# mwhittaker/frankenpaxos

Measured on NVIDIA H100. Metric: committed slots/sec (simulated) at 1M in-flight slots, higher is better.
Workload: dtype int32

## Files before the change

### frankenpaxos_b200/_lib.py

```python
import ctypes as C
import os

from . import build as _build

_lib = None

SYMBOLS = [
    "fpx_abi_version", "fpx_strerror", "fpx_last_error", "fpx_create", "fpx_destroy", "fpx_reset",
    "fpx_proxyleader_arm", "fpx_acceptor_phase2a", "fpx_proxyleader_phase2b", "fpx_replica_chosen",
    "fpx_chosen_watermark", "fpx_quorum_eval", "fpx_snapshot_acceptor", "fpx_snapshot_log",
    "fpx_proxyleader_arm_dev", "fpx_acceptor_phase2a_dev", "fpx_proxyleader_phase2b_dev",
    "fpx_replica_chosen_dev", "fpx_replica_chosen_last_dev", "fpx_chosen_watermark_dev", "fpx_sync",
    "fpx_stream", "fpx_launch_count", "fpx_set_coop_ctas_per_sm", "fpx_step_dev", "fpx_step_kernel_ms", "fpx_step_arm_ms",
    "fpx_acceptor_phase1a", "fpx_leader_safe_values",
    "fpx_vm_client_request", "fpx_vm_phase2a", "fpx_vm_learn_chosen", "fpx_vm_skip", "fpx_vm_client_request_dev", "fpx_vm_phase2a_dev", "fpx_vm_step_dev",
    "fpx_mencius_arm_range", "fpx_mencius_acceptor_noop_range", "fpx_mencius_range_phase2b",
    "fpx_mencius_replica_chosen_range", "fpx_mencius_replica_range_first", "fpx_mencius_replica_range_fill",
    "fpx_wire_decode_inbound", "fpx_wire_decode_inbound_dev", "fpx_wire_encode_phase2b", "fpx_wire_encode_phase2b_dev",
    "fpx_wire_encode_nack", "fpx_wire_encode_chosen",
    "fpx_step_submit", "fpx_step_wait", "fpx_retire_below", "fpx_exchange_export", "fpx_exchange_attach", "fpx_exchange_attach_local", "fpx_exchange_epoch",
    "fpx_global_watermark", "fpx_global_watermark_dev",
    "fpx_conflict_index_create", "fpx_conflict_index_destroy", "fpx_conflict_index_put_snapshot", "fpx_conflict_index_batch",
    "fpx_depgraph_create", "fpx_depgraph_destroy", "fpx_depgraph_commit", "fpx_depgraph_update_executed", "fpx_depgraph_execute",
    "fpx_epaxos_stream", "fpx_epaxos_sync", "fpx_epaxos_lead_dev", "fpx_epaxos_preaccept_dev", "fpx_epaxos_accept_dev",
# ... 75 lines not shown
    L.fpx_wire_encode_nack.argtypes = [vp, vp, i32, vp, i32, vp, p(i64)]; L.fpx_wire_encode_nack.restype = i32
    L.fpx_wire_encode_chosen.argtypes = [vp, vp, i32, vp, vp, i32, vp, i32, vp, p(i64)]
    L.fpx_wire_encode_chosen.restype = i32
    L.fpx_step_dev.argtypes = [vp, vp, i32, vp, i32, vp, vp, vp, i32, vp, vp, i32]; L.fpx_step_dev.restype = i32
    L.fpx_vm_step_dev.argtypes = [vp, vp, i32, vp, i32, vp, vp, i32, vp, vp]; L.fpx_vm_step_dev.restype = i32
    L.fpx_step_kernel_ms.argtypes = [vp, i32, p(C.c_float), p(C.c_float)]; L.fpx_step_kernel_ms.restype = i32
    L.fpx_step_arm_ms.argtypes = [vp, i32, p(C.c_float)]; L.fpx_step_arm_ms.restype = i32
    L.fpx_sync.argtypes = [vp, p(SyncResult)]; L.fpx_sync.restype = i32
    L.fpx_set_coop_ctas_per_sm.argtypes = [vp, i32]; L.fpx_set_coop_ctas_per_sm.restype = i32
    L.fpx_stream.argtypes = [vp]; L.fpx_stream.restype = vp
    L.fpx_launch_count.argtypes = [vp]; L.fpx_launch_count.restype = i64
    L.fpx_retire_below.argtypes = [vp, i32]; L.fpx_retire_below.restype = i32
    L.fpx_step_submit.argtypes = [vp, vp, i32, vp, i32, vp, i32, vp, vp, vp]; L.fpx_step_submit.restype = i32
    L.fpx_step_wait.argtypes = [vp, p(i32), p(i32), p(i32), p(i32), p(i64)]; L.fpx_step_wait.restype = i32
    L.fpx_exchange_export.argtypes = [vp, vp]; L.fpx_exchange_export.restype = i32
    L.fpx_exchange_attach.argtypes = [vp, i32, vp]; L.fpx_exchange_attach.restype = i32
    L.fpx_exchange_attach_local.argtypes = [vp, i32, vp]; L.fpx_exchange_attach_local.restype = i32
    L.fpx_exchange_epoch.argtypes = [vp]; L.fpx_exchange_epoch.restype = C.c_uint32
    L.fpx_global_watermark_dev.argtypes = [vp, C.c_uint32, i32, vp, vp]; L.fpx_global_watermark_dev.restype = i32
    L.fpx_global_watermark.argtypes = [vp, C.c_uint32, i32, p(i32), vp]; L.fpx_global_watermark.restype = i32
    if hasattr(L, "fpx_debug_set_tally_path"):
        L.fpx_debug_set_tally_path.argtypes = [vp, i32]; L.fpx_debug_set_tally_path.restype = i32
        L.fpx_debug_last_tally_path.argtypes = [vp]; L.fpx_debug_last_tally_path.restype = i32
    if L.fpx_abi_version() != 1:
        raise ImportError("libfpx.so ABI version mismatch")
    _lib = L
    return L
```

### frankenpaxos_b200/csrc/fpx_acceptor.cuh

```cuda
#pragma once
#include "fpx_common.cuh"

namespace fpx {

struct VoteConflict { int32_t dst, slot; };

struct AcceptorParams {
  Geometry g;
  const int4* in;
  int32_t n;
  int4* out_p2b;
  int2* out_nack;
  unsigned long long* votes;
  int32_t* acc_round;
  int32_t* acc_max_voted;
  uint32_t* accept_bits;
  int32_t* g_agg;
  uint32_t* g_wacc;
  uint32_t parity;
  int32_t append;
  DevStatus* st;
  VoteConflict* conflicts;
};

constexpr int kAccUnroll = 4;
#ifndef FPX_AT
#define FPX_AT 1024
#endif
constexpr int kAT = FPX_AT;
constexpr int kAW = kAT / 32;
__device__ __forceinline__ int grp_of(int dst) { return dst >> 16; }

__device__ __forceinline__ int decode_p2a(const Geometry& g, const int4& rec, int& key, int& loc, int& vix) {
  key = -1; loc = -1; vix = -1;
  int grp = rec.w >> 16, acc = rec.w & 0xffff;
  if ((uint32_t)grp >= (uint32_t)g.groups || acc >= g.per_group) return FPX_ERR_BAD_ACCEPTOR;
  if ((uint32_t)rec.y > (uint32_t)FPX_MAX_ROUND) return FPX_ERR_ROUND_RANGE;
  int l = local_slot(g, rec.x);
  if (l < 0 && l != kLocalRetired) return FPX_ERR_SLOT_RANGE;
  int v = voter_index(g, grp, acc, rec.x);
  if (v < 0 || (g.protocol == FPX_MENCIUS && grp != expected_group(g, rec.x))) return FPX_ERR_BAD_ACCEPTOR;
  key = grp * g.per_group + acc; loc = l; vix = v;
  return 0;
}
__device__ __forceinline__ int decode_key(const Geometry& g, const int4& rec) {
  int grp = rec.w >> 16, acc = rec.w & 0xffff;
  if ((uint32_t)grp >= (uint32_t)g.groups || acc >= g.per_group) return -1;
  if ((uint32_t)rec.y > (uint32_t)FPX_MAX_ROUND) return -1;
  return grp * g.per_group + acc;
}
__device__ __noinline__ void acceptor_error(DevStatus* st, int code, int index) { report_error(st, code, index); }

template <bool kExact>
__device__ __forceinline__ void acceptor_apply(const AcceptorParams& P, int4* out_p2b, int2* out_nack, int wlo, int whi,
                                               int lane, int run, uint32_t pos_base, int* s_mv, uint32_t& wacc,
                                               uint32_t& wnack) {
  const Geometry& g = P.g;
  const unsigned full = 0xffffffffu;
  const unsigned long long pol_out = l2_policy_evict_first();
  for (int base = wlo; base < whi; base += 32 * kAccUnroll) {
    int4 rec[kAccUnroll];
    unsigned long long cell[kAccUnroll], old[kAccUnroll];
#pragma unroll
    for (int u = 0; u < kAccUnroll; ++u) {
      int i = base + u * 32 + lane;
      rec[u] = (i < whi) ? ld_cg(P.in + i) : make_int4(0, -1, 0, -1);
      cell[u] = 0; old[u] = 0;
    }
#pragma unroll
    for (int u = 0; u < kAccUnroll; ++u) {
      const int i0 = base + u * 32;
      if (i0 >= whi) break;
      const int i = i0 + lane;
      int key, loc, vix;
      bool valid = false;
      if (i < whi) {
        int err = decode_p2a(g, rec[u], key, loc, vix);
        if (err && !kExact) acceptor_error(P.st, err, i);
        valid = err == 0;
      }
      const int r = rec[u].y;
      int mn = __reduce_min_sync(full, valid ? r : INT_MAX);
      int mx = __reduce_max_sync(full, valid ? r : INT_MIN);
      if (mx == INT_MIN) {
        if (!kExact && lane == 0) P.accept_bits[i0 >> 5] = 0;
        continue;
      }
      int my_run = __shfl_sync(full, run, key & 31);
      int cur;
// ... 36 lines not shown
        uint32_t before = pos_base + wacc + __popc(b & lanemask_lt());
        if (accept) {
          st_stream(out_p2b + before, make_int4(rec[u].w >> 16, rec[u].w & 0xffff, rec[u].x, r));
        } else if (valid) {
          int ldr = r % g.num_leaders;
          if (g.protocol == FPX_MENCIUS) ldr += (grp_of(rec[u].w) / g.agroups) * g.num_leaders;
          st_stream2(out_nack + ((uint32_t)i - before), make_int2(ldr, cur));
        }
      }
      wacc += __popc(b);
    }
    if (!kExact) {
#pragma unroll
      for (int u = 0; u < kAccUnroll; ++u) {
        if ((old[u] >> 32) == (cell[u] >> 32) && old[u] != cell[u]) {
          uint32_t cidx = atomicAdd(&P.st->n_conflicts, 1u);
          if (cidx < (uint32_t)kMaxConflicts) P.conflicts[cidx] = VoteConflict{rec[u].w, rec[u].x};
        }
      }
    }
  }
}

__global__ void __launch_bounds__(kAT, 1024 / kAT) acceptor_phase2a_kernel(AcceptorParams P) {
  const Geometry& g = P.g;
  extern __shared__ int s_mv[];
  __shared__ int s_wagg[kAW][kMaxKeys];
  __shared__ int s_tmp[kAW][kMaxKeys];
  __shared__ int s_win;

  const unsigned full = 0xffffffffu;
  const int tid = threadIdx.x, lane = tid & 31, warp = tid >> 5;
  const int total_warps = gridDim.x * kAW;
  const int per = (((P.n + total_warps - 1) / total_warps) + 31) & ~31;
  const int gw = blockIdx.x * kAW + warp;
  const int wlo = (int)min((long long)P.n, (long long)gw * per);
  const int whi = (int)min((long long)P.n, (long long)wlo + per);
  uint32_t* nack_ctr = P.parity ? &P.st->nack_total : &P.st->pad[0];
  uint32_t* nack_other = P.parity ? &P.st->pad[0] : &P.st->nack_total;
  if (blockIdx.x == 0 && tid == 0) *nack_other = 0;
  const uint32_t base_p2b = P.append ? (uint32_t)__ldcg(&P.st->n_p2b) : 0u;
  const uint32_t base_nack = P.append ? (uint32_t)__ldcg(&P.st->n_nack) : 0u;
  int4* const out_p2b = P.out_p2b + base_p2b;
  int2* const out_nack = P.out_nack + base_nack;
  for (int k = 0; k < g.num_keys; ++k) s_mv[k * kAT + tid] = INT_MIN;
  FPX_MARK(P.st->t_acceptor, 0);

  const unsigned long long pol_keep = l2_policy_evict_last();
  int wagg = INT_MIN;
  for (int base = wlo; base < whi; base += 32 * kAccUnroll) {
    int4 rec[kAccUnroll];
#pragma unroll
    for (int u = 0; u < kAccUnroll; ++u) {
      int i = base + u * 32 + lane;
      rec[u] = (i < whi) ? ld_keep(P.in + i, pol_keep) : make_int4(0, -1, 0, -1);
    }
#pragma unroll
    for (int u = 0; u < kAccUnroll; ++u) {
      if (base + u * 32 >= whi) break;
      const int key = decode_key(g, rec[u]);
      const bool valid = key >= 0;
      const int r = rec[u].y;
      int mn = __reduce_min_sync(full, valid ? r : INT_MAX);
      int mx = __reduce_max_sync(full, valid ? r : INT_MIN);
      if (mx == INT_MIN) continue;
      if (mn == mx) {
        unsigned present = __reduce_or_sync(full, valid ? (1u << key) : 0u);
        if ((present >> lane) & 1u) wagg = max(wagg, mx);
      } else {
        unsigned remaining = __ballot_sync(full, valid);
        while (remaining) {
          int leader = __ffs(remaining) - 1;
          int kk = __shfl_sync(full, key, leader);
          bool mine = valid && key == kk;
          int m = __reduce_max_sync(full, mine ? r : INT_MIN);
          if (lane == kk) wagg = max(wagg, m);
          remaining &= ~__ballot_sync(full, mine);
        }
      }
    }
  }
  s_wagg[warp][lane] = wagg;
  __syncthreads();
  int cta_agg = INT_MIN;
  if (warp == 0) {
#pragma unroll
    for (int w = 0; w < kAW; ++w) cta_agg = max(cta_agg, s_wagg[w][lane]);
    __stcg(&P.g_agg[blockIdx.x * kMaxKeys + lane], cta_agg);
  }
  FPX_MARK(P.st->t_acceptor, 1);
  grid_sync(P.st);
  FPX_MARK(P.st->t_acceptor, 2);

  for (int k = 0; k < g.num_keys; ++k) {
    int v = INT_MIN;
    for (int c = tid; c < (int)blockIdx.x; c += kAT) v = max(v, __ldcg(&P.g_agg[c * kMaxKeys + k]));
    v = __reduce_max_sync(full, v);
    if (lane == 0) s_tmp[warp][k] = v;
  }
  __syncthreads();
  int cta_carry = INT_MIN;
  if (lane < g.num_keys) {
    cta_carry = __ldcg(&P.acc_round[lane]);
#pragma unroll
    for (int w = 0; w < kAW; ++w) cta_carry = max(cta_carry, s_tmp[w][lane]);
  }
  int run = cta_carry;
  for (int w = 0; w < warp; ++w) run = max(run, s_wagg[w][lane]);

  FPX_MARK(P.st->t_acceptor, 3);
  uint32_t wacc = 0, wnack = 0;
  acceptor_apply<false>(P, out_p2b, out_nack, wlo, whi, lane, run, 0u, s_mv, wacc, wnack);
  if (lane == 0) {
    __stcg(&P.g_wacc[gw], wacc);
    if (wnack) atomicAdd(nack_ctr, wnack);
  }
  __syncthreads();
  for (int k = warp; k < g.num_keys; k += kAW) {
    int m = INT_MIN;
#pragma unroll
    for (int t = lane; t < kAT; t += 32) m = max(m, s_mv[k * kAT + t]);
    m = __reduce_max_sync(full, m);
    if (lane == 0 && m != INT_MIN) atomicMax(&P.acc_max_voted[k], m);
  }
  FPX_MARK(P.st->t_acceptor, 4);
  grid_sync(P.st);
  FPX_MARK(P.st->t_acceptor, 5);

  if (blockIdx.x == gridDim.x - 1 && warp == 0 && lane < g.num_keys) {
    int tot = cta_carry;
#pragma unroll
    for (int w = 0; w < kAW; ++w) tot = max(tot, s_wagg[w][lane]);
    P.acc_round[lane] = tot;
  }
  const uint32_t total_nacks = __ldcg(nack_ctr);
  if (total_nacks == 0) {
    if (blockIdx.x == 0 && tid == 0) { P.st->n_p2b = (int)base_p2b + P.n; P.st->n_nack = (int)base_nack; }
  } else {
    uint32_t before = 0;
    for (int j = lane; j < gw; j += 32) before += __ldcg(&P.g_wacc[j]);
    before = __reduce_add_sync(full, before);
    uint32_t wacc2 = 0, wnack2 = 0;
    acceptor_apply<true>(P, out_p2b, out_nack, wlo, whi, lane, run, before, s_mv, wacc2, wnack2);
    if (gw == (int)gridDim.x * kAW - 1 && lane == 0) {
      P.st->n_p2b = (int)(base_p2b + before + wacc2);
      P.st->n_nack = (int)base_nack + P.n - (int)(before + wacc2);
    }
  }

  if (blockIdx.x != 0) return;
  uint32_t nc = __ldcg(&P.st->n_conflicts);
  if (nc == 0) return;
  if (nc > (uint32_t)kMaxConflicts) {
    if (tid == 0) { report_error(P.st, FPX_ERR_CONFLICT, 0); P.st->n_conflicts = 0; }
    return;
  }
  for (uint32_t cix = 0; cix < nc; ++cix) {
    int dst = P.conflicts[cix].dst, slot = P.conflicts[cix].slot;
    if (tid == 0) s_win = -1;
    __syncthreads();
    for (int j = tid; j < P.n; j += kAT) {
      int4 rr = P.in[j];
      if (rr.w == dst && rr.x == slot && ((__ldcg(&P.accept_bits[j >> 5]) >> (j & 31)) & 1u)) atomicMax(&s_win, j);
    }
    __syncthreads();
    if (tid == 0 && s_win >= 0) {
      int4 rr = P.in[s_win];
      int l = local_slot(g, slot);
      int v = voter_index(g, dst >> 16, dst & 0xffff, slot);
// ... 9 lines not shown
```

### frankenpaxos_b200/csrc/fpx_arm.cuh

```cuda
#pragma once
#include "fpx_common.cuh"
#include "fpx_ranges.cuh"

namespace fpx {

struct ArmConflict { int32_t slot, round; };

struct ArmParams {
  Geometry g;
  PLState pl;
  const int4* in;
  int32_t n;
  DevStatus* st;
  ArmConflict* conflicts;
  uint32_t* win_bits;
  unsigned long long* votes;
  int32_t vanilla;
  RangeTable rng;
  int32_t check_rng;
};

__device__ __forceinline__ void note_arm_conflict(const ArmParams& P, int slot, int round) {
  uint32_t c = atomicAdd(&P.st->n_arm_conflicts, 1u);
  if (c < (uint32_t)kMaxConflicts) P.conflicts[c] = ArmConflict{slot, round};
// ... 83 lines not shown
        int i = (c0 + u) * 32 + lane;
        rec[u] = (c0 + u < n_chunks && i < P.n) ? ld_stream(P.in + i) : make_int4(-1, 0, 0, 0);
      }
#pragma unroll
      for (int u = 0; u < kArmUnroll; ++u) {
        int i = (c0 + u) * 32 + lane;
        local[u] = -1;
        old[u] = 0;
        if (c0 + u < n_chunks && i < P.n) {
          int l = local_slot(g, rec[u].x);
          if (l < 0) {
            if (l != kLocalRetired) report_error(P.st, FPX_ERR_SLOT_RANGE, i);
          } else if ((uint32_t)rec[u].y > (uint32_t)FPX_MAX_ROUND) {
            report_error(P.st, FPX_ERR_ROUND_RANGE, i);
          } else if (P.vanilla && rec[u].y != 0) {
            report_error(P.st, FPX_ERR_ROUND_RANGE, i);
          } else if (P.vanilla && ((rec[u].w >> 16) != 0 || (rec[u].w & 0xffff) >= g.per_group ||
                                   rec[u].x % g.per_group != (rec[u].w & 0xffff))) {
            report_error(P.st, FPX_ERR_BAD_ACCEPTOR, i);
          } else if (P.check_rng && range_find(P.rng, rec[u].x, rec[u].x + 1, rec[u].y) != nullptr) {
          } else {
            local[u] = l;
            want[u] = ((unsigned long long)(uint32_t)rec[u].z << 32) | (uint32_t)rec[u].y;
            old[u] = __ldcg((const unsigned long long*)(P.pl.rows + (size_t)l * g.row_words));
          }
        }
      }
    }
#pragma unroll
    for (int u = 0; u < kArmUnroll; ++u)
      if (local[u] >= 0 && old[u] == kU64Empty)
        old[u] = atomicCAS((unsigned long long*)(P.pl.rows + (size_t)local[u] * g.row_words), kU64Empty, want[u]);
#pragma unroll
    for (int u = 0; u < kArmUnroll; ++u) {
      if (c0 + u >= n_chunks) break;
      int i = (c0 + u) * 32 + lane;
      bool won = local[u] >= 0 && old[u] == kU64Empty;
      int self = -1;
      if (local[u] >= 0 && old[u] != kU64Empty) {
        const int4 rec = __ldcg(P.in + i);
        won = arm_finish(P, rec, old[u], i);
        self = rec.w & 0xffff;
      } else if (won && P.vanilla) {
        self = rel_to_slot(g, ring_to_rel(g, local[u])) % g.per_group;
      }
      if (won && P.vanilla) {
        uint32_t* row = P.pl.rows + (size_t)local[u] * g.row_words;
// ... 64 lines not shown
```

### frankenpaxos_b200/csrc/fpx_common.cuh

```cuda
#pragma once
#include <cuda_runtime.h>
#include <stdint.h>

#include "../../include/fpx.h"

namespace fpx {

constexpr uint32_t kUnarmed = 0xffffffffu;
constexpr uint32_t kDoneBit = 0x80000000u;
constexpr uint32_t kPoison = 0xfffffffeu;
constexpr uint32_t kBusy = 0xfffffffdu;
constexpr uint32_t kStampEmpty = 0xffffffffu;
constexpr uint64_t kU64Empty = ~0ull;
constexpr uint64_t kCellChosen = 0x8000000000000000ull;
constexpr int kThreads = 256;
constexpr int kWarps = kThreads / 32;
constexpr int kMaxKeys = FPX_MAX_ACCEPTORS;
constexpr int kMaxConflicts = 1024;
constexpr int kSms = 132;
constexpr int kMaxGrid = kSms * 8;
constexpr uint32_t kTsBadVoter = 1u, kTsAnomaly = 2u, kTsPoison = 4u, kTsVanillaRound = 8u;

struct DevStatus {
  unsigned long long err_word;
// ... 88 lines not shown
__device__ __forceinline__ unsigned long long l2_policy_evict_first() {
  unsigned long long pol;
  asm volatile("createpolicy.fractional.L2::evict_first.b64 %0, 1.0;" : "=l"(pol));
  return pol;
}
__device__ __forceinline__ void st_evict_first(int4* p, int4 v, unsigned long long pol) {
  asm volatile("st.global.L1::no_allocate.L2::cache_hint.v4.s32 [%0], {%1,%2,%3,%4}, %5;" ::"l"(p), "r"(v.x), "r"(v.y),
               "r"(v.z), "r"(v.w), "l"(pol));
}
__device__ __forceinline__ int4 ld_keep(const int4* p, unsigned long long pol) {
  int4 r;
  asm volatile("ld.global.nc.L1::no_allocate.L2::cache_hint.v4.s32 {%0,%1,%2,%3}, [%4], %5;"
               : "=r"(r.x), "=r"(r.y), "=r"(r.z), "=r"(r.w)
               : "l"(p), "l"(pol));
  return r;
}
__device__ __forceinline__ int4 ld_hint(const int4* p, unsigned long long pol) {
  int4 r;
  asm volatile("ld.global.L1::no_allocate.L2::cache_hint.v4.s32 {%0,%1,%2,%3}, [%4], %5;"
               : "=r"(r.x), "=r"(r.y), "=r"(r.z), "=r"(r.w)
               : "l"(p), "l"(pol));
  return r;
}
__device__ __forceinline__ void red_min_u32(uint32_t* p, uint32_t v) {
  asm volatile("red.global.min.u32 [%0], %1;" ::"l"(p), "r"(v) : "memory");
}
__device__ __forceinline__ void red_or_u32(uint32_t* p, uint32_t v) {
  asm volatile("red.global.or.b32 [%0], %1;" ::"l"(p), "r"(v) : "memory");
}
__device__ __forceinline__ void red_min_u64(unsigned long long* p, unsigned long long v) {
  asm volatile("red.global.min.u64 [%0], %1;" ::"l"(p), "l"(v) : "memory");
}
__device__ __forceinline__ void red_max_u64(unsigned long long* p, unsigned long long v) {
  asm volatile("red.global.max.u64 [%0], %1;" ::"l"(p), "l"(v) : "memory");
}
__device__ __forceinline__ void st_stream(int4* p, int4 v) {
  asm volatile("st.global.L1::no_allocate.v4.s32 [%0], {%1,%2,%3,%4};" ::"l"(p), "r"(v.x), "r"(v.y),
               "r"(v.z), "r"(v.w));
}
__device__ __forceinline__ void st_stream2(int2* p, int2 v) {
  asm volatile("st.global.L1::no_allocate.v2.s32 [%0], {%1,%2};" ::"l"(p), "r"(v.x), "r"(v.y));
}
__device__ __forceinline__ unsigned lanemask_lt() {
  unsigned m;
  asm("mov.u32 %0, %%lanemask_lt;" : "=r"(m));
  return m;
// ... 148 lines not shown
```

### frankenpaxos_b200/csrc/fpx_engine.cu

```cuda
#include <cuda_runtime.h>
#include <stdio.h>
#include <stdlib.h>
#include <string.h>

#include <algorithm>
#include <new>
#include <string>
#include <vector>

#include "fpx_acceptor.cuh"
#include "fpx_arm.cuh"
#include "fpx_common.cuh"
#include "fpx_conflict.cuh"
#include "fpx_depgraph.cuh"
#include "fpx_epaxos.cuh"
#include "fpx_ranges.cuh"
#include "fpx_replica_misc.cuh"
#include "fpx_tally.cuh"
#include "fpx_vanilla.cuh"
#include "fpx_wire.cuh"

using namespace fpx;

constexpr int kMaxEvents = 16;
// ... 16 lines not shown
  uint32_t vm_tag = 1;
  uint32_t* rng_tab = nullptr;
  int32_t rng_cap = 0;
  int32_t* rng_dec = nullptr;
  uint32_t rng_seq_base = 1;
  int unit_ranges = 0;
  cudaEvent_t* step_ev = nullptr;
  struct WireBuf { void* p = nullptr; size_t cap = 0; };
  WireBuf w_bytes, w_offs, w_kind, w_rec, w_out, w_tiles, w_arena, w_voffs;
  DevStatus* st = nullptr;
  DevExchange* xch = nullptr;
  DevExchange h_xch;
  unsigned long long* xch_table = nullptr;
  void* xch_opened[kMaxShards] = {};
  uint32_t xch_epoch = 0;
  int32_t* xch_out = nullptr;
  uint32_t* bits = nullptr;
  int32_t* g_agg = nullptr;
  uint32_t* g_wacc = nullptr;
  uint2* t_bw = nullptr;
  uint32_t* t_cc = nullptr;
  void* t_tmp = nullptr;
  int tally_path = 0;
  void* conflicts = nullptr;
  void* arm_conflicts = nullptr;
  uint32_t* arm_bits = nullptr;
  void* d_in = nullptr;
  void* d_out_a = nullptr;
  void* d_out_b = nullptr;
  DevStatus* h_st = nullptr;
  struct Lane {
    void *d_p2a = nullptr, *d_p2b = nullptr, *d_arm = nullptr, *d_out_p2b = nullptr, *d_out_nack = nullptr, *d_out_chosen = nullptr;
    cudaEvent_t ev_p2a = nullptr, ev_p2b = nullptr, ev_acc = nullptr, ev_done = nullptr, ev_d2h = nullptr;
    DevStatus* h_st = nullptr;
    fpx_p2b* out_p2b = nullptr; fpx_nack* out_nack = nullptr; fpx_chosen* out_chosen = nullptr;
    int32_t n_p2a = 0;
    bool busy = false;
  } lane[2];
  int lane_head = 0, lane_tail = 0, lanes_in_flight = 0;
  uint32_t parity = 0;
  int grid_acceptor = 0;
  int grid_tally = 0;
  int occ_acceptor = 0, occ_tally = 0;
  int tally_max_sub = 0;
  int num_sms = 0;
  uint32_t seq_base = 1;
// ... 179 lines not shown
  CKC(cudaStreamCreateWithFlags(&e->h2d_stream, cudaStreamNonBlocking));
  CKC(cudaStreamCreateWithFlags(&e->d2h_stream, cudaStreamNonBlocking));
  for (int i = 0; i < kMaxEvents; ++i) CKC(cudaEventCreateWithFlags(&e->ev[i], cudaEventDisableTiming));
  size_t mb = (size_t)cfg->max_batch;
  CKC(cudaMalloc(&e->rows, (size_t)g.local_slots * g.row_words * 4));
  if (g.ovf_cap) {
    CKC(cudaMalloc(&e->ovf_keys, (size_t)g.ovf_cap * 8));
    CKC(cudaMalloc(&e->ovf_rows, (size_t)g.ovf_cap * g.row_words * 4));
  }
  CKC(cudaMalloc(&e->votes, ((size_t)g.local_slots * g.voters * 8) << g.cell_shift));
  CKC(cudaMalloc(&e->acc_round, kMaxKeys * 4));
  CKC(cudaMalloc(&e->acc_max_voted, kMaxKeys * 4));
  CKC(cudaMalloc(&e->rlog, (size_t)g.local_slots * 8));
  if (cfg->protocol == FPX_MENCIUS) {
    e->rng_cap = std::max(1024, g.ovf_cap);
    CKC(cudaMalloc(&e->rng_tab, (size_t)e->rng_cap * kRangeWords * 4));
  }
  if (cfg->protocol != FPX_MULTIPAXOS) CKC(cudaMalloc(&e->rng_dec, (size_t)(FPX_MAX_RANGE_BATCH + 1) * 4));
  CKC(cudaMalloc(&e->st, sizeof(DevStatus)));
  CKC(cudaMalloc(&e->xch, sizeof(DevExchange)));
  CKC(cudaMalloc(&e->xch_table, kMaxShards * 8));
  CKC(cudaMalloc(&e->xch_out, (1 + kMaxShards) * 4));
  CKC(cudaMalloc(&e->bits, (mb / 32 + 2) * 4));
  CKC(cudaMalloc(&e->g_agg, (size_t)kMaxGrid * kMaxKeys * 4));
  CKC(cudaMalloc(&e->g_wacc, (size_t)kMaxGrid * kAW * 4));
  CKC(cudaMalloc(&e->t_bw, (mb / kChunkVotes + 2) * 32 * 8));
  CKC(cudaMalloc(&e->t_cc, (mb / kChunkVotes + 2) * 4));
  CKC(cudaMalloc(&e->t_tmp, (mb + kChunkVotes) * 8));
  {
    cudaDeviceProp prop;
    CKC(cudaGetDeviceProperties(&prop, cfg->device));
    if (!prop.cooperativeLaunch) return fail(FPX_ERR_UNSUPPORTED);
    e->num_sms = prop.multiProcessorCount;
    int occ = 0;
    CKC(cudaFuncSetAttribute(acceptor_phase2a_kernel, cudaFuncAttributeMaxDynamicSharedMemorySize,
                             kMaxKeys * kAT * 4));
    CKC(cudaOccupancyMaxActiveBlocksPerMultiprocessor(&occ, acceptor_phase2a_kernel, kAT,
                                                      (size_t)g.num_keys * kAT * 4));
    e->occ_acceptor = std::max(occ, 1);
    e->grid_acceptor = std::min(std::max(occ, 1) * e->num_sms, kMaxGrid);
    const int smem_cap = kTallySmem;
    e->tally_max_sub = (40 * 1024 / 4) * kChunkVotes;
    const void* tk = tally_kernel_ptr(g.row_words);
    CKC(cudaFuncSetAttribute(tk, cudaFuncAttributeMaxDynamicSharedMemorySize, smem_cap));
    CKC(cudaOccupancyMaxActiveBlocksPerMultiprocessor(&occ, tk, kTT, smem_cap));
    e->occ_tally = std::max(occ, 1);
    e->grid_tally = std::min(std::max(occ, 1) * e->num_sms, kMaxGrid);
  }
  CKC(cudaMalloc(&e->conflicts, kMaxConflicts * 8));
  CKC(cudaMalloc(&e->arm_conflicts, kMaxConflicts * 8));
  CKC(cudaMalloc(&e->arm_bits, (mb / 32 + 2) * 4));
  CKC(cudaMalloc(&e->d_in, mb * 16));
  CKC(cudaMalloc(&e->d_out_a, mb * 16));
  CKC(cudaMalloc(&e->d_out_b, mb * 8));
  CKC(cudaMallocHost(&e->h_st, sizeof(DevStatus)));
#undef CKC
  memset(&e->h_xch, 0, sizeof(e->h_xch));
  e->h_xch.n = g.shard_count <= kMaxShards ? g.shard_count : 0;
  e->h_xch.mine = g.shard_index;
  e->h_xch.tabs[g.shard_index < kMaxShards ? g.shard_index : 0] = g.shard_count <= kMaxShards ? e->xch_table : nullptr;
  e->h_xch.enabled = g.shard_count > 1 && g.shard_count <= kMaxShards;
// ... 68 lines not shown

int fpx_set_coop_ctas_per_sm(fpx_engine* e, int32_t ctas_per_sm) {
  if (!e || ctas_per_sm < 0) return FPX_ERR_INVALID_ARG;
  int a = ctas_per_sm == 0 ? e->occ_acceptor : std::min(e->occ_acceptor, ctas_per_sm);
  int t = ctas_per_sm == 0 ? e->occ_tally : std::min(e->occ_tally, ctas_per_sm);
  e->grid_acceptor = std::min(a * e->num_sms, kMaxGrid);
  e->grid_tally = std::min(t * e->num_sms, kMaxGrid);
  return FPX_OK;
}

int fpx_debug_phase_times(fpx_engine* e, unsigned long long* acceptor8, unsigned long long* tally8) {
  if (!e) return FPX_ERR_INVALID_ARG;
  CK(e, cudaStreamSynchronize(e->stream));
  CK(e, cudaMemcpy(acceptor8, e->st->t_acceptor, 64, cudaMemcpyDeviceToHost));
  CK(e, cudaMemcpy(tally8, e->st->t_tally, 64, cudaMemcpyDeviceToHost));
  return FPX_OK;
}
int64_t fpx_launch_count(const fpx_engine* e) { return e ? e->launches : 0; }
int fpx_debug_set_tally_path(fpx_engine* e, int32_t path) {
  if (!e || (path & ~6)) return FPX_ERR_INVALID_ARG;
  e->tally_path = path;
  return FPX_OK;
}
int fpx_debug_last_tally_path(fpx_engine* e) {
  if (!e) return FPX_ERR_INVALID_ARG;
  uint32_t v = 0;
  CK(e, cudaStreamSynchronize(e->stream));
  CK(e, cudaMemcpy(&v, &e->st->ts_path, 4, cudaMemcpyDeviceToHost));
  return (int)v;
}


static int check_n(fpx_engine* e, const void* p, int32_t n) {
  if (!e || n < 0 || n > e->cfg.max_batch || (n > 0 && !p)) return FPX_ERR_INVALID_ARG;
  return FPX_OK;
}

static ArmParams arm_params(fpx_engine* e, const fpx_p2a* d_in, int32_t n, int vanilla) {
  ArmParams P;
  P.g = e->g;
  P.pl = PLState{e->rows, e->ovf_keys, e->ovf_rows};
  P.in = (const int4*)d_in;
  P.n = n;
  P.st = e->st;
  P.conflicts = (ArmConflict*)e->arm_conflicts;
  P.win_bits = e->arm_bits;
// ... 33 lines not shown
  int c = check_n(e, d_in, n);
  if (c != FPX_OK) return c;
  if (n > 0 && (!d_out_p2b || !d_out_nack)) return FPX_ERR_INVALID_ARG;
  if (e->g.protocol == FPX_VANILLA_MENCIUS) return FPX_ERR_UNSUPPORTED;
  if (n == 0) {
    if (!append) CK(e, cudaMemsetAsync(&e->st->n_p2b, 0, 8, stream));
    return FPX_OK;
  }
  AcceptorParams P;
  P.g = e->g;
  P.in = (const int4*)d_in;
  P.n = n;
  P.out_p2b = (int4*)d_out_p2b;
  P.out_nack = (int2*)d_out_nack;
  P.votes = e->votes;
  P.acc_round = e->acc_round;
  P.acc_max_voted = e->acc_max_voted;
  P.accept_bits = e->bits;
  P.g_agg = e->g_agg;
  P.g_wacc = e->g_wacc;
  P.st = e->st;
  P.conflicts = (VoteConflict*)e->conflicts;
  int grid = std::max(1, std::min(e->grid_acceptor, (n + kAT - 1) / kAT));
  P.parity = e->parity;
  P.append = append;
  e->parity ^= 1u;
  void* args[] = {&P};
  CK(e, cudaLaunchCooperativeKernel((const void*)acceptor_phase2a_kernel, dim3(grid), dim3(kAT), args,
                                    (size_t)e->g.num_keys * kAT * 4, stream));
  e->launches++;
  CK(e, cudaGetLastError());
  return FPX_OK;
}

static int renormalize_rlog_if_needed(fpx_engine* e, int32_t bound);

static int tally_launch(fpx_engine* e, const fpx_p2b* d_in, int32_t n, fpx_chosen* d_out, int fuse, int32_t* d_wm) {
  int c = check_n(e, d_in, n);
  if (c != FPX_OK) return c;
  if (n > 0 && !d_out) return FPX_ERR_INVALID_ARG;
  e->last_p2b_n = n;
  if (n == 0) {
    CK(e, cudaMemsetAsync(&e->st->n_chosen, 0, 4, e->stream));
    return fuse ? fpx_chosen_watermark_dev(e, d_wm) : FPX_OK;
  }
  if (fuse) {
    c = renormalize_rlog_if_needed(e, 2 * n > n ? 2 * n : n);
    if (c != FPX_OK) return c;
  }
  if (e->seq_base > 0xffffffffu - (uint32_t)n - 16u) {
    size_t nrows = (size_t)e->g.local_slots;
    renormalize_stamps_kernel<<<(unsigned)((nrows + 255) / 256), 256, 0, e->stream>>>(e->g, e->rows, nrows);
// ... 617 lines not shown
```

### frankenpaxos_b200/engine.py

```python
import ctypes as C

import numpy as np

from . import _lib

P2A = np.dtype([("slot", "<i4"), ("round", "<i4"), ("value_id", "<i4"), ("dst", "<i4")])
P2B = np.dtype([("group", "<i4"), ("acceptor", "<i4"), ("slot", "<i4"), ("round", "<i4")])
CHOSEN = np.dtype([("slot", "<i4"), ("value_id", "<i4")])
NACK = np.dtype([("leader", "<i4"), ("round", "<i4")])
P2A_RANGE = np.dtype([("slot_start", "<i4"), ("slot_end", "<i4"), ("round", "<i4"), ("dst", "<i4")])
P2B_RANGE = np.dtype([("dst", "<i4"), ("slot_start", "<i4"), ("slot_end", "<i4"), ("round", "<i4")])
CHOSEN_RANGE = np.dtype([("slot_start", "<i4"), ("slot_end", "<i4")])
VM_SKIP = np.dtype([("server", "<i4"), ("slot_start", "<i4"), ("slot_stop", "<i4"), ("own", "<i4")])
VALUE_NOOP = -(1 << 31)
WIRE_REC = np.dtype([("a", "<i4"), ("b", "<i4"), ("c", "<i4"), ("d", "<i4")])
WIRE_PROXYLEADER_INBOUND, WIRE_ACCEPTOR_INBOUND = 0, 1
WIRE_MENCIUS_PROXYLEADER_INBOUND, WIRE_MENCIUS_ACCEPTOR_INBOUND = 2, 3

MULTIPAXOS, MENCIUS, VANILLA_MENCIUS = 0, 1, 2

OK = 0
ERR_INVALID_ARG, ERR_CONFIG, ERR_CUDA, ERR_UNKNOWN_SLOT_ROUND, ERR_BAD_ACCEPTOR = -1, -2, -3, -4, -5
ERR_SLOT_RANGE, ERR_ROUND_RANGE, ERR_OVERFLOW_FULL, ERR_CONFLICT, ERR_NO_DEVICE, ERR_UNSUPPORTED = \
    -6, -7, -8, -9, -10, -11
# ... 82 lines not shown
        return buf.raw

    def exchange_attach(self, shard, handle):
        self._check(self._L.fpx_exchange_attach(self.h, shard, C.c_char_p(bytes(handle))))

    def exchange_attach_local(self, shard, peer):
        self._check(self._L.fpx_exchange_attach_local(self.h, shard, peer.h))

    @property
    def exchange_epoch(self):
        return self._L.fpx_exchange_epoch(self.h)

    def global_watermark(self, epoch=None, timeout_ms=5000):
        n = self.cfg.shard_count
        fr = np.empty(n, dtype=np.int32)
        out = C.c_int32(0)
        ep = self.exchange_epoch if epoch is None else epoch
        self._check(self._L.fpx_global_watermark(self.h, ep, timeout_ms, C.byref(out), fr.ctypes.data))
        return out.value, fr

    def set_tally_path(self, exact):
        self._check(self._L.fpx_debug_set_tally_path(self.h, 2 if exact else 0))

    @property
    def last_tally_path(self):
        return {1: "sweep", 2: "exact"}.get(self._L.fpx_debug_last_tally_path(self.h), "none")

    def proxyleader_arm(self, p2a):
        p2a = np.ascontiguousarray(p2a, dtype=P2A)
        err = C.c_int64(-1)
        st = self._L.fpx_proxyleader_arm(self.h, p2a.ctypes.data, len(p2a), C.byref(err))
        self._check(st, err.value)

    def acceptor_phase2a(self, p2a):
        p2a = np.ascontiguousarray(p2a, dtype=P2A)
        n = len(p2a)
        out = np.empty(max(n, 1), dtype=P2B)
        nack = np.empty(max(n, 1), dtype=NACK)
        n1, n2, err = C.c_int32(0), C.c_int32(0), C.c_int64(-1)
        st = self._L.fpx_acceptor_phase2a(self.h, p2a.ctypes.data, n, out.ctypes.data, C.byref(n1),
                                          nack.ctypes.data, C.byref(n2), C.byref(err))
        self._check(st, err.value)
        return out[:n1.value], nack[:n2.value]

    def proxyleader_phase2b(self, p2b):
        p2b = np.ascontiguousarray(p2b, dtype=P2B)
# ... 231 lines not shown
```

### profiles/exp_step.py

```python
import argparse
import ctypes
import json
import os
import sys

import numpy as np
import torch

ROOT = os.path.dirname(os.path.dirname(os.path.abspath(__file__)))
sys.path.insert(0, ROOT)
ap = argparse.ArgumentParser()
ap.add_argument("--steps", type=int, default=12)
ap.add_argument("--variants", default="default,acc_first,exact,default,acc_first")
ap.add_argument("--out", default="")
ap.add_argument("--old-lib", action="store_true", help="time the round-1 build (profiles/_r1/libfpx.so) instead")
ap.add_argument("--lib", default="", help="time another build of libfpx.so (tuning variants under profiles/_var/)")
args = ap.parse_args()
if args.old_lib:
    os.environ["FPX_LIB_OVERRIDE"] = os.path.join(ROOT, "profiles", "_r1", "libfpx.so")
if args.lib:
    os.environ["FPX_LIB_OVERRIDE"] = os.path.join(ROOT, args.lib)

import bench
from frankenpaxos_b200 import Engine, traces as T
# ... 1 lines not shown
cfg = bench.CFG
n = 1 << 20
S = args.steps + 3
dev = torch.device("cuda")


def td(x):
    return torch.from_numpy(x.view(np.int32).reshape(len(x), -1)).to(dev)


base = [T.workload(b, cfg, n) for b in range(4)]
outp = torch.empty((3 * n, 4), dtype=torch.int32, device=dev)
outn = torch.empty((3 * n, 2), dtype=torch.int32, device=dev)
outc = torch.empty((3 * n, 2), dtype=torch.int32, device=dev)
wm = torch.zeros(1, dtype=torch.int32, device=dev)
results = {}
for variant in args.variants.split(","):
    eng = Engine(slot_capacity=S * n, max_batch=3 * n, overflow_capacity=1 << 10, **cfg)
    L = eng._L
    L.fpx_debug_phase_times.argtypes = [ctypes.c_void_p, ctypes.c_void_p, ctypes.c_void_p]
    ext = torch.cuda.ExternalStream(eng.stream, device=dev)
    if not args.old_lib:
        eng._check(L.fpx_debug_set_tally_path(eng.h, sum(bit for tok, bit in (("exact", 2), ("nored", 4)) if tok in variant.split("_"))))
    flush = torch.empty(1 << 28, dtype=torch.uint8, device=dev) if "flush" in variant else None
    ins = []
    for s in range(S):
        a, p, b = base[s % 4]
        def rb(r):
            o = r.copy(); o["slot"] = o["slot"] + s * n; return o
        ins.append((td(rb(a)), td(rb(p)), td(rb(b))))
    torch.cuda.synchronize()
    names = ["arm", "acceptor", "tally", "replica", "watermark"]
    order = ["acceptor", "arm", "tally", "replica", "watermark"] if "accfirst" in variant.split("_") else names
    evs = [[torch.cuda.Event(enable_timing=True) for _ in range(6)] for _ in range(S)]

    def run(which, s):
        da, dp, db = ins[s]
        if which == "arm": eng.proxyleader_arm_dev(da.data_ptr(), n)
        elif which == "acceptor": eng.acceptor_phase2a_dev(dp.data_ptr(), 3 * n, outp.data_ptr(), outn.data_ptr())
        elif which == "tally":
            if flush is not None:
                with torch.cuda.stream(ext):
                    flush.view(torch.int64).sum()
                evs[s][order.index("tally")].record(ext)
            eng.proxyleader_phase2b_dev(db.data_ptr(), 3 * n, outc.data_ptr())
        elif which == "replica": eng.replica_chosen_last_dev(outc.data_ptr())
# ... 55 lines not shown
```

Measured before the change: 3.046 billion.

## Segment acceptor scan/apply passes so input stays L2-resident between passes

The cooperative acceptor kernel used to scan the entire input, grid-sync, then apply over the entire input, so the second pass re-read data that had already been evicted from L2. The input is now split into up to 8 segments sized to about half of L2, with a scan/sync/apply cycle per segment. Per-segment running maxima are kept in extra shared memory and per-segment accept counts are kept so the exact nack path can still be replayed. Input loads switch to an evict-first hint and the arm header loads use evict-last. The cost is one extra grid-wide sync per segment and more dynamic shared memory, which may lower occupancy.

New measurement: 3.515 billion, median of 6. 15.4% higher.

```diff
diff --git a/frankenpaxos_b200/_lib.py b/frankenpaxos_b200/_lib.py
--- a/frankenpaxos_b200/_lib.py
+++ b/frankenpaxos_b200/_lib.py
@@ -121,6 +121,8 @@
     if hasattr(L, "fpx_debug_set_tally_path"):
         L.fpx_debug_set_tally_path.argtypes = [vp, i32]; L.fpx_debug_set_tally_path.restype = i32
         L.fpx_debug_last_tally_path.argtypes = [vp]; L.fpx_debug_last_tally_path.restype = i32
+    if hasattr(L, "fpx_debug_set_acceptor_segments"):
+        L.fpx_debug_set_acceptor_segments.argtypes = [vp, i32]; L.fpx_debug_set_acceptor_segments.restype = i32
     if L.fpx_abi_version() != 1:
         raise ImportError("libfpx.so ABI version mismatch")
     _lib = L
diff --git a/frankenpaxos_b200/csrc/fpx_acceptor.cuh b/frankenpaxos_b200/csrc/fpx_acceptor.cuh
--- a/frankenpaxos_b200/csrc/fpx_acceptor.cuh
+++ b/frankenpaxos_b200/csrc/fpx_acceptor.cuh
@@ -1,4 +1,6 @@
 #pragma once
+#include <algorithm>
+
 #include "fpx_common.cuh"
 
 namespace fpx {
@@ -17,6 +19,7 @@
   uint32_t* accept_bits;
   int32_t* g_agg;
   uint32_t* g_wacc;
+  int32_t segments;
   uint32_t parity;
   int32_t append;
   DevStatus* st;
@@ -29,6 +32,13 @@
 #endif
 constexpr int kAT = FPX_AT;
 constexpr int kAW = kAT / 32;
+constexpr int kAccMaxSegments = 8;
+inline int acceptor_segments(long long n, long long l2_bytes) {
+  const long long seg_bytes = l2_bytes / 2;
+  if (seg_bytes <= 0) return 1;
+  const long long s = (n * 16 + seg_bytes - 1) / seg_bytes;
+  return (int)std::max(1ll, std::min((long long)kAccMaxSegments, s));
+}
 __device__ __forceinline__ int grp_of(int dst) { return dst >> 16; }
 
 __device__ __forceinline__ int decode_p2a(const Geometry& g, const int4& rec, int& key, int& loc, int& vix) {
@@ -64,7 +74,7 @@
 #pragma unroll
     for (int u = 0; u < kAccUnroll; ++u) {
       int i = base + u * 32 + lane;
-      rec[u] = (i < whi) ? ld_cg(P.in + i) : make_int4(0, -1, 0, -1);
+      rec[u] = (i < whi) ? ld_hint(P.in + i, pol_out) : make_int4(0, -1, 0, -1);
       cell[u] = 0; old[u] = 0;
     }
 #pragma unroll
@@ -147,30 +157,9 @@
   }
 }
 
-__global__ void __launch_bounds__(kAT, 1024 / kAT) acceptor_phase2a_kernel(AcceptorParams P) {
+__device__ __forceinline__ int acceptor_scan(const AcceptorParams& P, int wlo, int whi, int lane) {
   const Geometry& g = P.g;
-  extern __shared__ int s_mv[];
-  __shared__ int s_wagg[kAW][kMaxKeys];
-  __shared__ int s_tmp[kAW][kMaxKeys];
-  __shared__ int s_win;
-
   const unsigned full = 0xffffffffu;
-  const int tid = threadIdx.x, lane = tid & 31, warp = tid >> 5;
-  const int total_warps = gridDim.x * kAW;
-  const int per = (((P.n + total_warps - 1) / total_warps) + 31) & ~31;
-  const int gw = blockIdx.x * kAW + warp;
-  const int wlo = (int)min((long long)P.n, (long long)gw * per);
-  const int whi = (int)min((long long)P.n, (long long)wlo + per);
-  uint32_t* nack_ctr = P.parity ? &P.st->nack_total : &P.st->pad[0];
-  uint32_t* nack_other = P.parity ? &P.st->pad[0] : &P.st->nack_total;
-  if (blockIdx.x == 0 && tid == 0) *nack_other = 0;
-  const uint32_t base_p2b = P.append ? (uint32_t)__ldcg(&P.st->n_p2b) : 0u;
-  const uint32_t base_nack = P.append ? (uint32_t)__ldcg(&P.st->n_nack) : 0u;
-  int4* const out_p2b = P.out_p2b + base_p2b;
-  int2* const out_nack = P.out_nack + base_nack;
-  for (int k = 0; k < g.num_keys; ++k) s_mv[k * kAT + tid] = INT_MIN;
-  FPX_MARK(P.st->t_acceptor, 0);
-
   const unsigned long long pol_keep = l2_policy_evict_last();
   int wagg = INT_MIN;
   for (int base = wlo; base < whi; base += 32 * kAccUnroll) {
@@ -205,41 +194,91 @@
       }
     }
   }
-  s_wagg[warp][lane] = wagg;
-  __syncthreads();
-  int cta_agg = INT_MIN;
-  if (warp == 0) {
-#pragma unroll
-    for (int w = 0; w < kAW; ++w) cta_agg = max(cta_agg, s_wagg[w][lane]);
-    __stcg(&P.g_agg[blockIdx.x * kMaxKeys + lane], cta_agg);
-  }
-  FPX_MARK(P.st->t_acceptor, 1);
-  grid_sync(P.st);
-  FPX_MARK(P.st->t_acceptor, 2);
-
-  for (int k = 0; k < g.num_keys; ++k) {
-    int v = INT_MIN;
-    for (int c = tid; c < (int)blockIdx.x; c += kAT) v = max(v, __ldcg(&P.g_agg[c * kMaxKeys + k]));
-    v = __reduce_max_sync(full, v);
-    if (lane == 0) s_tmp[warp][k] = v;
-  }
-  __syncthreads();
-  int cta_carry = INT_MIN;
-  if (lane < g.num_keys) {
-    cta_carry = __ldcg(&P.acc_round[lane]);
-#pragma unroll
-    for (int w = 0; w < kAW; ++w) cta_carry = max(cta_carry, s_tmp[w][lane]);
-  }
-  int run = cta_carry;
-  for (int w = 0; w < warp; ++w) run = max(run, s_wagg[w][lane]);
-
-  FPX_MARK(P.st->t_acceptor, 3);
-  uint32_t wacc = 0, wnack = 0;
-  acceptor_apply<false>(P, out_p2b, out_nack, wlo, whi, lane, run, 0u, s_mv, wacc, wnack);
-  if (lane == 0) {
-    __stcg(&P.g_wacc[gw], wacc);
-    if (wnack) atomicAdd(nack_ctr, wnack);
-  }
+  return wagg;
+}
+
+__device__ __forceinline__ void acceptor_range(int n, int seg_len, int per, int s, int gw, int& lo, int& hi) {
+  const long long s_lo = min((long long)n, (long long)s * seg_len), s_hi = min((long long)n, s_lo + seg_len);
+  lo = (int)min(s_hi, s_lo + (long long)gw * per);
+  hi = (int)min(s_hi, (long long)lo + per);
+}
+
+__global__ void __launch_bounds__(kAT, 1024 / kAT) acceptor_phase2a_kernel(AcceptorParams P) {
+  const Geometry& g = P.g;
+  extern __shared__ int s_acc_dyn[];
+  int* const s_mv = s_acc_dyn;
+  int* const s_run = s_acc_dyn + g.num_keys * kAT;
+  __shared__ int s_wagg[kAW][kMaxKeys];
+  __shared__ int s_tmp[2][kAW][kMaxKeys];
+  __shared__ int s_win;
+
+  const unsigned full = 0xffffffffu;
+  const int tid = threadIdx.x, lane = tid & 31, warp = tid >> 5;
+  const int total_warps = gridDim.x * kAW;
+  const int S = P.segments;
+  const int seg_len = S == 1 ? P.n : (((P.n + S - 1) / S) + 31) & ~31;
+  const int per = (((seg_len + total_warps - 1) / total_warps) + 31) & ~31;
+  const int gw = blockIdx.x * kAW + warp;
+  uint32_t* nack_ctr = P.parity ? &P.st->nack_total : &P.st->pad[0];
+  uint32_t* nack_other = P.parity ? &P.st->pad[0] : &P.st->nack_total;
+  if (blockIdx.x == 0 && tid == 0) *nack_other = 0;
+  const uint32_t base_p2b = P.append ? (uint32_t)__ldcg(&P.st->n_p2b) : 0u;
+  const uint32_t base_nack = P.append ? (uint32_t)__ldcg(&P.st->n_nack) : 0u;
+  int4* const out_p2b = P.out_p2b + base_p2b;
+  int2* const out_nack = P.out_nack + base_nack;
+  for (int k = 0; k < g.num_keys; ++k) s_mv[k * kAT + tid] = INT_MIN;
+  FPX_MARK(P.st->t_acceptor, 0);
+
+  int wlo, whi;
+  acceptor_range(P.n, seg_len, per, 0, gw, wlo, whi);
+  int wagg = acceptor_scan(P, wlo, whi, lane);
+  int prev = lane < g.num_keys ? __ldcg(&P.acc_round[lane]) : INT_MIN;
+  uint32_t wnack = 0;
+  for (int s = 0; s < S; ++s) {
+    if (s > 0) __syncthreads();
+    s_wagg[warp][lane] = wagg;
+    __syncthreads();
+    int32_t* const agg = P.g_agg + (s & 1) * kMaxGrid * kMaxKeys;
+    if (warp == 0) {
+      int cta_agg = INT_MIN;
+#pragma unroll
+      for (int w = 0; w < kAW; ++w) cta_agg = max(cta_agg, s_wagg[w][lane]);
+      __stcg(&agg[blockIdx.x * kMaxKeys + lane], cta_agg);
+    }
+    if (s == 0) FPX_MARK(P.st->t_acceptor, 1);
+    grid_sync(P.st);
+    if (s == 0) FPX_MARK(P.st->t_acceptor, 2);
+
+    for (int k = 0; k < g.num_keys; ++k) {
+      int vb = INT_MIN, va = INT_MIN;
+      for (int c = tid; c < (int)gridDim.x; c += kAT) {
+        const int v = __ldcg(&agg[c * kMaxKeys + k]);
+        va = max(va, v);
+        if (c < (int)blockIdx.x) vb = max(vb, v);
+      }
+      vb = __reduce_max_sync(full, vb);
+      va = __reduce_max_sync(full, va);
+      if (lane == 0) { s_tmp[0][warp][k] = vb; s_tmp[1][warp][k] = va; }
+    }
+    __syncthreads();
+    int run = prev;
+    if (lane < g.num_keys) {
+#pragma unroll
+      for (int w = 0; w < kAW; ++w) { run = max(run, s_tmp[0][w][lane]); prev = max(prev, s_tmp[1][w][lane]); }
+    }
+    for (int w = 0; w < warp; ++w) run = max(run, s_wagg[w][lane]);
+    s_run[s * kAT + tid] = run;
+    if (s == 0) FPX_MARK(P.st->t_acceptor, 3);
+
+    uint32_t wacc = 0;
+    acceptor_apply<false>(P, out_p2b, out_nack, wlo, whi, lane, run, 0u, s_mv, wacc, wnack);
+    if (lane == 0) __stcg(&P.g_wacc[s * total_warps + gw], wacc);
+    if (s + 1 < S) {
+      acceptor_range(P.n, seg_len, per, s + 1, gw, wlo, whi);
+      wagg = acceptor_scan(P, wlo, whi, lane);
+    }
+  }
+  if (lane == 0 && wnack) atomicAdd(nack_ctr, wnack);
   __syncthreads();
   for (int k = warp; k < g.num_keys; k += kAW) {
     int m = INT_MIN;
@@ -252,24 +291,26 @@
   grid_sync(P.st);
   FPX_MARK(P.st->t_acceptor, 5);
 
-  if (blockIdx.x == gridDim.x - 1 && warp == 0 && lane < g.num_keys) {
-    int tot = cta_carry;
-#pragma unroll
-    for (int w = 0; w < kAW; ++w) tot = max(tot, s_wagg[w][lane]);
-    P.acc_round[lane] = tot;
-  }
+  if (blockIdx.x == gridDim.x - 1 && warp == 0 && lane < g.num_keys) P.acc_round[lane] = prev;
   const uint32_t total_nacks = __ldcg(nack_ctr);
   if (total_nacks == 0) {
     if (blockIdx.x == 0 && tid == 0) { P.st->n_p2b = (int)base_p2b + P.n; P.st->n_nack = (int)base_nack; }
   } else {
     uint32_t before = 0;
-    for (int j = lane; j < gw; j += 32) before += __ldcg(&P.g_wacc[j]);
-    before = __reduce_add_sync(full, before);
-    uint32_t wacc2 = 0, wnack2 = 0;
-    acceptor_apply<true>(P, out_p2b, out_nack, wlo, whi, lane, run, before, s_mv, wacc2, wnack2);
-    if (gw == (int)gridDim.x * kAW - 1 && lane == 0) {
-      P.st->n_p2b = (int)(base_p2b + before + wacc2);
-      P.st->n_nack = (int)base_nack + P.n - (int)(before + wacc2);
+    int j0 = 0;
+    for (int s = 0; s < S; ++s) {
+      const int idx = s * total_warps + gw;
+      uint32_t b = 0;
+      for (int j = j0 + lane; j < idx; j += 32) b += __ldcg(&P.g_wacc[j]);
+      before += __reduce_add_sync(full, b);
+      j0 = idx;
+      acceptor_range(P.n, seg_len, per, s, gw, wlo, whi);
+      uint32_t wacc2 = 0, wnack2 = 0;
+      acceptor_apply<true>(P, out_p2b, out_nack, wlo, whi, lane, s_run[s * kAT + tid], before, s_mv, wacc2, wnack2);
+      if (s == S - 1 && gw == total_warps - 1 && lane == 0) {
+        P.st->n_p2b = (int)(base_p2b + before + wacc2);
+        P.st->n_nack = (int)base_nack + P.n - (int)(before + wacc2);
+      }
     }
   }
 
diff --git a/frankenpaxos_b200/csrc/fpx_arm.cuh b/frankenpaxos_b200/csrc/fpx_arm.cuh
--- a/frankenpaxos_b200/csrc/fpx_arm.cuh
+++ b/frankenpaxos_b200/csrc/fpx_arm.cuh
@@ -129,7 +129,8 @@
           } else {
             local[u] = l;
             want[u] = ((unsigned long long)(uint32_t)rec[u].z << 32) | (uint32_t)rec[u].y;
-            old[u] = __ldcg((const unsigned long long*)(P.pl.rows + (size_t)l * g.row_words));
+            const unsigned long long* hdr = (const unsigned long long*)(P.pl.rows + (size_t)l * g.row_words);
+            old[u] = P.vanilla ? __ldcg(hdr) : ld_u64_evict_last(hdr);
           }
         }
       }
diff --git a/frankenpaxos_b200/csrc/fpx_common.cuh b/frankenpaxos_b200/csrc/fpx_common.cuh
--- a/frankenpaxos_b200/csrc/fpx_common.cuh
+++ b/frankenpaxos_b200/csrc/fpx_common.cuh
@@ -134,6 +134,14 @@
                : "l"(p), "l"(pol));
   return r;
 }
+__device__ __forceinline__ unsigned long long ld_u64_evict_last(const unsigned long long* p) {
+  unsigned long long v;
+  asm volatile("{ .reg .b64 pol; createpolicy.fractional.L2::evict_last.b64 pol, 1.0; "
+               "ld.global.cg.L2::cache_hint.u64 %0, [%1], pol; }"
+               : "=l"(v) : "l"(p));
+  return v;
+}
+
 __device__ __forceinline__ void red_min_u32(uint32_t* p, uint32_t v) {
   asm volatile("red.global.min.u32 [%0], %1;" ::"l"(p), "r"(v) : "memory");
 }
diff --git a/frankenpaxos_b200/csrc/fpx_engine.cu b/frankenpaxos_b200/csrc/fpx_engine.cu
--- a/frankenpaxos_b200/csrc/fpx_engine.cu
+++ b/frankenpaxos_b200/csrc/fpx_engine.cu
@@ -62,6 +62,8 @@
   uint32_t* t_cc = nullptr;
   void* t_tmp = nullptr;
   int tally_path = 0;
+  int acc_segments = 0;
+  long long l2_bytes = 0;
   void* conflicts = nullptr;
   void* arm_conflicts = nullptr;
   uint32_t* arm_bits = nullptr;
@@ -287,8 +289,8 @@
   CKC(cudaMalloc(&e->xch_table, kMaxShards * 8));
   CKC(cudaMalloc(&e->xch_out, (1 + kMaxShards) * 4));
   CKC(cudaMalloc(&e->bits, (mb / 32 + 2) * 4));
-  CKC(cudaMalloc(&e->g_agg, (size_t)kMaxGrid * kMaxKeys * 4));
-  CKC(cudaMalloc(&e->g_wacc, (size_t)kMaxGrid * kAW * 4));
+  CKC(cudaMalloc(&e->g_agg, (size_t)2 * kMaxGrid * kMaxKeys * 4));
+  CKC(cudaMalloc(&e->g_wacc, (size_t)kAccMaxSegments * kMaxGrid * kAW * 4));
   CKC(cudaMalloc(&e->t_bw, (mb / kChunkVotes + 2) * 32 * 8));
   CKC(cudaMalloc(&e->t_cc, (mb / kChunkVotes + 2) * 4));
   CKC(cudaMalloc(&e->t_tmp, (mb + kChunkVotes) * 8));
@@ -297,11 +299,12 @@
     CKC(cudaGetDeviceProperties(&prop, cfg->device));
     if (!prop.cooperativeLaunch) return fail(FPX_ERR_UNSUPPORTED);
     e->num_sms = prop.multiProcessorCount;
+    e->l2_bytes = prop.l2CacheSize;
     int occ = 0;
     CKC(cudaFuncSetAttribute(acceptor_phase2a_kernel, cudaFuncAttributeMaxDynamicSharedMemorySize,
-                             kMaxKeys * kAT * 4));
+                             (kMaxKeys + kAccMaxSegments) * kAT * 4));
     CKC(cudaOccupancyMaxActiveBlocksPerMultiprocessor(&occ, acceptor_phase2a_kernel, kAT,
-                                                      (size_t)g.num_keys * kAT * 4));
+                                                      (size_t)(g.num_keys + kAccMaxSegments) * kAT * 4));
     e->occ_acceptor = std::max(occ, 1);
     e->grid_acceptor = std::min(std::max(occ, 1) * e->num_sms, kMaxGrid);
     const int smem_cap = kTallySmem;
@@ -416,6 +419,11 @@
   e->tally_path = path;
   return FPX_OK;
 }
+int fpx_debug_set_acceptor_segments(fpx_engine* e, int32_t segments) {
+  if (!e || segments < 0 || segments > kAccMaxSegments) return FPX_ERR_INVALID_ARG;
+  e->acc_segments = segments;
+  return FPX_OK;
+}
 int fpx_debug_last_tally_path(fpx_engine* e) {
   if (!e) return FPX_ERR_INVALID_ARG;
   uint32_t v = 0;
@@ -495,12 +503,13 @@
   P.st = e->st;
   P.conflicts = (VoteConflict*)e->conflicts;
   int grid = std::max(1, std::min(e->grid_acceptor, (n + kAT - 1) / kAT));
+  P.segments = e->acc_segments > 0 ? e->acc_segments : acceptor_segments(n, e->l2_bytes);
   P.parity = e->parity;
   P.append = append;
   e->parity ^= 1u;
   void* args[] = {&P};
   CK(e, cudaLaunchCooperativeKernel((const void*)acceptor_phase2a_kernel, dim3(grid), dim3(kAT), args,
-                                    (size_t)e->g.num_keys * kAT * 4, stream));
+                                    (size_t)(e->g.num_keys + P.segments) * kAT * 4, stream));
   e->launches++;
   CK(e, cudaGetLastError());
   return FPX_OK;
diff --git a/frankenpaxos_b200/engine.py b/frankenpaxos_b200/engine.py
--- a/frankenpaxos_b200/engine.py
+++ b/frankenpaxos_b200/engine.py
@@ -128,6 +128,9 @@
     def set_tally_path(self, exact):
         self._check(self._L.fpx_debug_set_tally_path(self.h, 2 if exact else 0))
 
+    def set_acceptor_segments(self, segments):
+        self._check(self._L.fpx_debug_set_acceptor_segments(self.h, segments))
+
     @property
     def last_tally_path(self):
         return {1: "sweep", 2: "exact"}.get(self._L.fpx_debug_last_tally_path(self.h), "none")
diff --git a/profiles/exp_step.py b/profiles/exp_step.py
--- a/profiles/exp_step.py
+++ b/profiles/exp_step.py
@@ -47,6 +47,9 @@
     ext = torch.cuda.ExternalStream(eng.stream, device=dev)
     if not args.old_lib:
         eng._check(L.fpx_debug_set_tally_path(eng.h, sum(bit for tok, bit in (("exact", 2), ("nored", 4)) if tok in variant.split("_"))))
+    for tok in variant.split("_"):
+        if tok.startswith("seg"):
+            eng.set_acceptor_segments(int(tok[3:]))
     flush = torch.empty(1 << 28, dtype=torch.uint8, device=dev) if "flush" in variant else None
     ins = []
     for s in range(S):
```
